# gpmp-dev/gpmp

Measured on AMD Instinct MI355X. Metric: fp64 predict+NLL throughput (points/s) and potrf TFLOP/s vs roofline, n=32k, higher is better.
Workload: dtype f64

## Files before the change

gpmp_amd/csrc/common.h:

```cpp
#pragma once
#include <hip/hip_runtime.h>
#include <cstdint>
#include <cstdio>
#include <cstring>
#include <atomic>
#include <vector>
#include "../../include/gpmp_hip.h"

namespace gpmp {

typedef double d4 __attribute__((ext_vector_type(4)));
typedef double d2 __attribute__((ext_vector_type(2)));

constexpr int NB = GPMP_NB;
constexpr int OUTER_BLOCKS = 4;

void set_error(const char* fmt, ...);
int hip_fail(hipError_t e, const char* what);

#define GPMP_HIP_TRY(expr)                                   \
  do {                                                       \
    hipError_t e__ = (expr);                                 \
    if (e__ != hipSuccess) return ::gpmp::hip_fail(e__, #expr); \
  } while (0)

#define GPMP_ARG(cond, k, msg)                                          \
  do {                                                                  \
    if (!(cond)) { ::gpmp::set_error("argument %d: %s", (k), (msg)); return -(k); } \
  } while (0)

inline hipStream_t as_stream(gpmp_stream_t s) { return reinterpret_cast<hipStream_t>(s); }

hipError_t stage_vector(std::vector<double>* v, double* dst, hipStream_t st);

int device_cu_count();

struct DeviceOnce {
  std::atomic<unsigned long long> mask{0};
  long long need() {
    int dev = 0;
    if (hipGetDevice(&dev) != hipSuccess || dev < 0 || dev > 62) return -1;
    const unsigned long long bit = 1ull << dev;
    return (mask.load(std::memory_order_acquire) & bit) ? 0 : (long long)bit;
  }
  void done(long long bit) { mask.fetch_or((unsigned long long)bit, std::memory_order_release); }
};

enum ProfKind { PK_GEMM_NT = 0, PK_GEMM_NN = 1, PK_GEMM_TN = 2, PK_GEMM_TT = 3, PK_POTF2 = 4, PK_GRAM = 5,
                PK_COLDOTS = 6, PK_GRAD = 7, PK_GEMM2_NT = 8, PK_GEMM2_NN = 9, PK_GEMM2_TN = 10, PK_GEMM2_TT = 11,
                PK_COUNT = 12 };
extern bool g_prof_on;
void prof_start(int kind, hipStream_t st);
void prof_stop(int kind, hipStream_t st, double work);
struct ProfScope {
  int kind; hipStream_t st; double work; bool on;
  ProfScope(int k, hipStream_t s, double w) : kind(k), st(s), work(w), on(g_prof_on) { if (on) prof_start(kind, st); }
  ~ProfScope() { if (on) prof_stop(kind, st, work); }
};

struct GemmOpts {
  int lower_only = 0;
  int kstart_row = 0;
  int kend_row = 0;
  int kstart_col = 0;
  int kend_col = 0;
  int batch = 1;
  long stride_a = 0, stride_b = 0, stride_c = 0;
  int batch2 = 1;
  long stride2_a = 0, stride2_b = 0, stride2_c = 0;
  int lean = 0;
  int stair_num = 0, stair_den = 0, stair_off = 0, stair_sub = 0;
  int kg_rnum = 0, kg_rden = 0, kg_roff = 0, kg_cnum = 0, kg_cden = 0, kg_coff = 0;
};
int launch_gemm(bool a_kc, bool b_kc, int M, int N, int K, double alpha, const double* A, long lda,
                const double* B, long ldb, double beta, double* C, long ldc, const GemmOpts& o,
                hipStream_t st);

int launch_trsm_leaf_forward(const double* L, long ldl, const double* dinv_leaf, int nb, double* B, long ldb, int ncols,
                             double* G, hipStream_t st);

int launch_potf2_inv(double* A, long lda, int jb, double* dinv, int* info_dev, int offset, hipStream_t st);
int launch_potf2_inv_batch(double* A, long lda, int jb, double* dinv, int* info_dev, int offset, int nprob, long stride_a,
                           long stride_dinv, hipStream_t st);
int launch_trtri_blocks(const double* L, long ldl, int n, double* dinv, hipStream_t st);

constexpr int TRSV_FEW_MAX = 16;
int trsv_few(const double* L, int n, long ldl, const double* dinv, double* B, int m, long ldb, int trans,
             hipStream_t st);

int launch_tril(double* A, int n, long lda, hipStream_t st, int nprob = 1, long prob_stride = 0);
int launch_symmetrize(double* A, int n, long lda, hipStream_t st);
int launch_diag_blocks(double* T, int n, long ldt, const double* dinv, hipStream_t st, int nprob = 1, long prob_stride_t = 0,
                       long prob_stride_dinv = 0);

struct ProblemBatch {
  int nprob = 1;
  long stride_a = 0;
  long stride_dinv = 0;
};
int potrf_blocked_batch(double* A, int n, long lda, double* dinv, int* info_dev, const ProblemBatch& pb, hipStream_t st);
int trtri_doubling_batch(const double* L, int n, long ldl, const double* dinv, double* T, long ldt, const ProblemBatch& pb,
                         long stride_t, hipStream_t st);
int launch_gram_lower_batch(const double* x, long stride_x, const int* ns_dev, int nmax, int d, int p, const double* theta_host,
                            int noise, double diag_add, double* K, long ldk, long stride_k, int nprob, hipStream_t st,
                            const double* pp_dev = nullptr);
int gram_param_block_elems();
void fill_gram_param_block(double* blk, int d, int p, const double* theta, int noise, double diag_add);
int launch_grad_trace_batch(const double* Kinv, long ldk, long stride_kinv, const double* x, long stride_x, const int* ns_dev, int nmax,
                            int d, int p, const double* theta_host, int noise, const double* F, const double* G, int r, long ldf,
                            long stride_f, double* g_dev, double* ws, int nprob, hipStream_t st, const double* pp_dev = nullptr);
int lauum_lower_batch(const double* T, int n, long ldt, long stride_t, double* Kinv, long ldk, long stride_k, int nprob,
                      hipStream_t st);

}
```

gpmp_amd/csrc/gemm_f64.hip:

```cpp
#include "common.h"
#include <cstdlib>

namespace gpmp {

int g_machine_busy = 0;

namespace {

constexpr int BM = 128, BN = 128, BK = 16;
constexpr int LDK = 18;
constexpr int LDN = 144;
constexpr int TILE = 2304;
constexpr int NXCD = 8;
typedef unsigned int v4u __attribute__((ext_vector_type(4)));

struct GemmParams {
  const double* A;
  const double* B;
  double* C;
  long lda, ldb, ldc;
  int M, N, K;
  double alpha, beta;
  int lower_only, kstart_row, kend_row, kend_col;
  int kstart_col;
// ... 646 lines not shown
      const int k0 = kt * BK;
      double* sa = smem + buf * 2 * V2_TILE;
      double* sb = sa + V2_TILE;
#pragma unroll
      for (int s = 0; s < 4; ++s)
        __builtin_amdgcn_raw_ptr_buffer_load_lds(rsA, (lds_ptr)(sa + (wave * 32 + s * 8) * 16), 16, voffA[s & 1],
                                                 ((wave * 32 + s * 8) * (int)p.ldg + k0) * 8, 0, 0);
#pragma unroll
      for (int s = 0; s < 4; ++s)
        __builtin_amdgcn_raw_ptr_buffer_load_lds(rsB, (lds_ptr)(sb + (wave * 4 + s) * 128), 16, voffB[s & 1],
                                                 ((k0 + wave * 4 + s) * (int)p.ldb) * 8, 0, 0);
    };
    auto read_frags = [&](int ks, int buf) {
      const double* sa = smem + buf * 2 * V2_TILE;
      const double* sb = sa + V2_TILE;
#pragma unroll
      for (int i = 0; i < MI; ++i) fa[ks][i] = sa[v2_frag_addr<true>(wm + i * 16 + lr, ks * 4 + lk)];
#pragma unroll
      for (int j = 0; j < NJ; ++j) fb[ks][j] = sb[v2_frag_addr<false>(wn + j * 16 + lr, ks * 4 + lk)];
    };
    auto mfma_step = [&](int ks) {
#pragma unroll
      for (int i = 0; i < MI; ++i)
#pragma unroll
        for (int j = 0; j < NJ; ++j)
          acc[i][j] = __builtin_amdgcn_mfma_f64_16x16x4f64(fa[ks][i], fb[ks][j], acc[i][j], 0, 0, 0);
    };
#pragma unroll
    for (int i = 0; i < MI; ++i)
#pragma unroll
      for (int j = 0; j < NJ; ++j) acc[i][j] = (d4){0.0, 0.0, 0.0, 0.0};

    issue(0, 0);
    __syncthreads();
    read_frags(0, 0);
    read_frags(1, 0);
    for (int kt = 0; kt < nk; ++kt) {
      const int cur = kt & 1;
      const bool more = kt + 1 < nk;
      if (more) issue(kt + 1, cur ^ 1);
      read_frags(2, cur);
      __builtin_amdgcn_sched_barrier(0);
      mfma_step(0);
      __builtin_amdgcn_sched_barrier(0);
      read_frags(3, cur);
      __builtin_amdgcn_sched_barrier(0);
      mfma_step(1);
      mfma_step(2);
      __builtin_amdgcn_sched_barrier(0);
      __syncthreads();
      if (more) {
        read_frags(0, cur ^ 1);
        read_frags(1, cur ^ 1);
      }
      __builtin_amdgcn_sched_barrier(0);
      mfma_step(3);
    }
    double* cb = strip + (long)jb * BM * p.ldb;
    if (ncv == BNW) {
#pragma unroll
      for (int i = 0; i < MI; ++i)
#pragma unroll
        for (int r = 0; r < 4; ++r) {
          double* rp = cb + (long)(i * 16 + 4 * r) * p.ldb;
#pragma unroll
          for (int j = 0; j < NJ; ++j) rp[lane_off + j * 16] = acc[i][j][r];
        }
    } else {
#pragma unroll
      for (int i = 0; i < MI; ++i)
#pragma unroll
        for (int r = 0; r < 4; ++r) {
          double* rp = cb + (long)(i * 16 + 4 * r) * p.ldb;
#pragma unroll
          for (int j = 0; j < NJ; ++j)
            if (wn + j * 16 + lr < ncv) rp[lane_off + j * 16] = acc[i][j][r];
        }
    }
    __threadfence_block();
    __syncthreads();
  }
}

struct LeafGParams {
  const double* L;
  long ldl;
  const double* dinv;
  double* G;
  long ldg;
};

__global__ void __launch_bounds__(256) build_leaf_g_kernel(LeafGParams p) {
  const int jb = blockIdx.x, ib = blockIdx.y;
  if (ib > jb) return;
  const int t = threadIdx.x;
  const double* __restrict__ D = p.dinv + (size_t)jb * BM * BM;
  double* __restrict__ out = p.G + (long)jb * BM * p.ldg + ib * BN;
  if (ib == jb) {
    for (int e = t; e < BM * BN / 2; e += 256) {
      const int r = e / (BN / 2), c = (e % (BN / 2)) * 2;
      *reinterpret_cast<d2*>(out + (long)r * p.ldg + c) = *reinterpret_cast<const d2*>(D + r * BM + c);
    }
    return;
  }
  const double* __restrict__ Lb = p.L + (long)jb * BM * p.ldl + ib * BN;
  const int lane = t & 63, wave = t >> 6;
  const int wm = (wave >> 1) * 64, wn = (wave & 1) * 64;
  const int lr = lane & 15, lk = lane >> 4;
  d4 acc[4][4];
#pragma unroll
  for (int i = 0; i < 4; ++i)
#pragma unroll
    for (int j = 0; j < 4; ++j) acc[i][j] = (d4){0.0, 0.0, 0.0, 0.0};
  for (int k0 = 0; k0 < BM; k0 += 4) {
    double a[4], b[4];
#pragma unroll
    for (int i = 0; i < 4; ++i) a[i] = D[(wm + i * 16 + lr) * BM + k0 + lk];
#pragma unroll
    for (int j = 0; j < 4; ++j) b[j] = Lb[(long)(k0 + lk) * p.ldl + wn + j * 16 + lr];
#pragma unroll
    for (int i = 0; i < 4; ++i)
#pragma unroll
      for (int j = 0; j < 4; ++j) acc[i][j] = __builtin_amdgcn_mfma_f64_16x16x4f64(a[i], b[j], acc[i][j], 0, 0, 0);
  }
#pragma unroll
  for (int i = 0; i < 4; ++i)
#pragma unroll
    for (int r = 0; r < 4; ++r)
#pragma unroll
      for (int j = 0; j < 4; ++j)
        out[(long)(wm + i * 16 + lk + 4 * r) * p.ldg + wn + j * 16 + lr] = -acc[i][j][r];
}

constexpr int SBM = 32, SBN = 128, SLD = 18;

template <int SBMT>
__global__ void __launch_bounds__(256) gemm_nt_small_kernel(GemmParams p) {
  __shared__ __attribute__((aligned(16))) double sA[2][SBMT * SLD];
  __shared__ __attribute__((aligned(16))) double sB[2][SBN * SLD];
  const int row0 = blockIdx.y * SBMT, col0 = blockIdx.x * SBN;
  if (p.lower_only && col0 > row0 + SBMT - 1) return;
  __builtin_amdgcn_s_setprio(3);
  const int t = threadIdx.x, lane = t & 63;
  const int wave = __builtin_amdgcn_readfirstlane(t >> 6);
  const int wn = wave * 32;
  const int lr = lane & 15, lk = lane >> 4;
  const int srow = t >> 2, skq = (t & 3) * 4;
  const bool has_a = t < 4 * SBMT;
  int ar = row0 + (has_a ? srow : 0), br0 = col0 + srow, br1 = col0 + srow + 64;
  ar = ar < p.M ? ar : p.M - 1;
  br0 = br0 < p.N ? br0 : p.N - 1;
  br1 = br1 < p.N ? br1 : p.N - 1;
  const double* __restrict__ ap = p.A + (long)ar * p.lda + skq;
  const double* __restrict__ bp0 = p.B + (long)br0 * p.ldb + skq;
  const double* __restrict__ bp1 = p.B + (long)br1 * p.ldb + skq;

  constexpr int MI = SBMT / 16;
  d4 acc[MI][2];
#pragma unroll
  for (int i = 0; i < MI; ++i)
#pragma unroll
    for (int j = 0; j < 2; ++j) acc[i][j] = (d4){0.0, 0.0, 0.0, 0.0};

  const int nk = p.K / BK;
  for (int kc = 0; kc < nk; kc += 8) {
    const int cnt = (nk - kc) < 8 ? (nk - kc) : 8;
    d2 ra[8][2], rb[8][4];
#pragma unroll
    for (int q = 0; q < 8; ++q) {
      if (q < cnt) {
        const int ko = (kc + q) * BK;
        if (has_a) {
          ra[q][0] = *reinterpret_cast<const d2*>(ap + ko);
          ra[q][1] = *reinterpret_cast<const d2*>(ap + ko + 2);
        }
        rb[q][0] = *reinterpret_cast<const d2*>(bp0 + ko);
        rb[q][1] = *reinterpret_cast<const d2*>(bp0 + ko + 2);
// ... 123 lines not shown
          double v = alpha * acc[i][j][r];
          if (beta != 0.0) v += beta * *cp;
          *cp = v;
        }
      }
    }
}

#pragma clang diagnostic pop

template <bool AKC, bool BKC, bool CACC>
int launch_t(const GemmParams& p, hipStream_t st) {
  static DeviceOnce attr_once;
  const size_t lds = sizeof(double) * 4 * TILE;
  const size_t lds2 = sizeof(double) * 4 * V2_TILE;
  if (const long long dev_bit = attr_once.need()) {
    if (dev_bit < 0) { set_error("hipGetDevice failed or device ordinal above 62"); return -1; }
    GPMP_HIP_TRY(hipFuncSetAttribute(reinterpret_cast<const void*>(gemm_f64_kernel<AKC, BKC, CACC>),
                                     hipFuncAttributeMaxDynamicSharedMemorySize, (int)lds));
    GPMP_HIP_TRY(hipFuncSetAttribute(reinterpret_cast<const void*>(gemm_f64_kernel_v2<AKC, BKC, CACC>),
                                     hipFuncAttributeMaxDynamicSharedMemorySize, (int)lds2));
    GPMP_HIP_TRY(hipFuncSetAttribute(reinterpret_cast<const void*>(gemm_f64_kernel_v2<AKC, BKC, CACC, 112>),
                                     hipFuncAttributeMaxDynamicSharedMemorySize, (int)lds2));
    GPMP_HIP_TRY(hipFuncSetAttribute(reinterpret_cast<const void*>(gemm_f64_kernel_v2<AKC, BKC, CACC, 96>),
                                     hipFuncAttributeMaxDynamicSharedMemorySize, (int)lds2));
    attr_once.done(dev_bit);
  }
  static int use_v2 = -1;
  if (use_v2 < 0) { const char* e = getenv("GPMP_GEMM_V2"); use_v2 = e ? atoi(e) : 1; }
  const bool v2ok = use_v2 && p.K >= 512 && p.aligned && (p.M % 2 == 0) && (p.N % 2 == 0) && (p.K % BK == 0) && p.K > 0 &&
                    ((reinterpret_cast<uintptr_t>(p.C) & 15) == 0) && (p.ldc % 2 == 0) &&
                    (p.lda % 2 == 0) && (p.ldb % 2 == 0) && (p.ldc >= p.N) &&
                    ((long)BM * p.lda * 8 + (long)p.K * 8 < 0x7FFFFFFFL) && ((long)BN * p.ldb * 8 + (long)p.K * 8 < 0x7FFFFFFFL);
  GemmParams pf = p;
  if (v2ok && p.batch == 1 && p.batch2 == 1 && !p.lower_only && !p.stair_den && !(p.kstart_row | p.kend_row | p.kstart_col | p.kend_col | p.kg_rden | p.kg_cden) && p.N >= 16 * BN) {
    const long slots = 2L * device_cu_count();
    auto cost = [&](int w) { const long t = (long)p.tiles_m * ((p.N + w - 1) / w); return ((t + slots - 1) / slots) * (long)w; };
    long best = cost(BN);
    for (int w : {112, 96}) {
      const long c = cost(w);
      if (c * 100 < best * 97) { best = c; pf.bn = w; }
    }
    if (pf.bn != BN) {
      pf.tiles_n = (p.N + pf.bn - 1) / pf.bn;
      pf.ntiles = pf.tiles_m * pf.tiles_n;
    }
  }
  constexpr int small_max = 128;
  const bool lean_nt = p.batch == 1 && p.batch2 == 1 && AKC && BKC && p.lean && p.aligned && (p.K % BK == 0) && p.K >= BK && p.K <= 512 &&
                       !(p.kstart_row | p.kend_row | p.kstart_col | p.kend_col) && ((long)SBN * p.ldb * 8 + (long)p.K * 8 < 0x7FFFFFFFL) &&
                       ((long)SBM * p.lda * 8 + (long)p.K * 8 < 0x7FFFFFFFL);
  const bool small_nt = !lean_nt && p.batch == 1 && p.batch2 == 1 && AKC && BKC && p.aligned && (p.K % BK == 0) && p.K >= BK && p.K <= 512 &&
                        p.ntiles <= (p.K >= 512 ? 384 : small_max) && !(p.kstart_row | p.kend_row | p.kstart_col | p.kend_col);
  {
    const double kavg = (p.kstart_row || p.kend_row || p.kstart_col || p.kend_col || p.kg_rden || p.kg_cden) ? 0.5 * p.K : (double)p.K;
    ProfScope ps((AKC ? (BKC ? PK_GEMM_NT : PK_GEMM_NN) : (BKC ? PK_GEMM_TT : PK_GEMM_TN)) + ((v2ok && !small_nt) ? 8 : 0), st,
                 (!p.lower_only && !p.stair_den && !(p.kstart_row | p.kend_row | p.kstart_col | p.kend_col | p.kg_rden | p.kg_cden))
                     ? 2.0 * (double)p.M * (double)p.N * (double)p.K * p.batch * p.batch2
                     : 2.0 * (double)p.ntiles * BM * BN * kavg * p.batch * p.batch2);
    if (lean_nt) hipLaunchKernelGGL(gemm_nt_lean_kernel, dim3((p.N + SBN - 1) / SBN, (p.M + SBM - 1) / SBM), dim3(256), 0, st, p);
    else if (small_nt) {
      constexpr long below16 = 160;
      const long wg32 = (long)((p.N + SBN - 1) / SBN) * ((p.M + SBM - 1) / SBM);
      if (wg32 < below16) hipLaunchKernelGGL(gemm_nt_small_kernel<16>, dim3((p.N + SBN - 1) / SBN, (p.M + 15) / 16), dim3(256), 0, st, p);
      else hipLaunchKernelGGL(gemm_nt_small_kernel<SBM>, dim3((p.N + SBN - 1) / SBN, (p.M + SBM - 1) / SBM), dim3(256), 0, st, p);
    }
    else if (v2ok && pf.bn == 112) hipLaunchKernelGGL((gemm_f64_kernel_v2<AKC, BKC, CACC, 112>), dim3(pf.ntiles, pf.batch, pf.batch2), dim3(256), lds2, st, pf);
    else if (v2ok && pf.bn == 96) hipLaunchKernelGGL((gemm_f64_kernel_v2<AKC, BKC, CACC, 96>), dim3(pf.ntiles, pf.batch, pf.batch2), dim3(256), lds2, st, pf);
    else if (v2ok) hipLaunchKernelGGL((gemm_f64_kernel_v2<AKC, BKC, CACC>), dim3(p.ntiles, p.batch, p.batch2), dim3(256), lds2, st, p);
    else hipLaunchKernelGGL((gemm_f64_kernel<AKC, BKC, CACC>), dim3(p.ntiles, p.batch, p.batch2), dim3(256), lds, st, p);
  }
  GPMP_HIP_TRY(hipGetLastError());
  return 0;
}

template <bool AKC, bool BKC>
int launch_c(const GemmParams& p, hipStream_t st) {
  if (p.beta != 0.0 && p.alpha != 0.0) return launch_t<AKC, BKC, true>(p, st);
  return launch_t<AKC, BKC, false>(p, st);
}

}

int launch_trsm_leaf_forward(const double* L, long ldl, const double* dinv_leaf, int nb, double* B, long ldb, int ncols,
                             double* G, hipStream_t st) {
  if (ncols <= 0) return 0;
  const long ldg = (long)nb * BN;
  {
    LeafGParams g{L, ldl, dinv_leaf, G, ldg};
    hipLaunchKernelGGL(build_leaf_g_kernel, dim3(nb, nb), dim3(256), 0, st, g);
    GPMP_HIP_TRY(hipGetLastError());
  }
  static DeviceOnce attr_once;
  const size_t lds2 = sizeof(double) * 4 * V2_TILE;
  if (const long long dev_bit = attr_once.need()) {
    if (dev_bit < 0) { set_error("hipGetDevice failed or device ordinal above 62"); return -1; }
    GPMP_HIP_TRY(hipFuncSetAttribute(reinterpret_cast<const void*>(trsm_leaf_kernel<128>),
                                     hipFuncAttributeMaxDynamicSharedMemorySize, (int)lds2));
    GPMP_HIP_TRY(hipFuncSetAttribute(reinterpret_cast<const void*>(trsm_leaf_kernel<64>),
                                     hipFuncAttributeMaxDynamicSharedMemorySize, (int)lds2));
    GPMP_HIP_TRY(hipFuncSetAttribute(reinterpret_cast<const void*>(trsm_leaf_kernel<32>),
                                     hipFuncAttributeMaxDynamicSharedMemorySize, (int)lds2));
    GPMP_HIP_TRY(hipFuncSetAttribute(reinterpret_cast<const void*>(trsm_leaf_kernel<16>),
                                     hipFuncAttributeMaxDynamicSharedMemorySize, (int)lds2));
    GPMP_HIP_TRY(hipFuncSetAttribute(reinterpret_cast<const void*>(trsm_leaf_kernel<112>),
                                     hipFuncAttributeMaxDynamicSharedMemorySize, (int)lds2));
    GPMP_HIP_TRY(hipFuncSetAttribute(reinterpret_cast<const void*>(trsm_leaf_kernel<96>),
                                     hipFuncAttributeMaxDynamicSharedMemorySize, (int)lds2));
    GPMP_HIP_TRY(hipFuncSetAttribute(reinterpret_cast<const void*>(trsm_leaf_kernel<80>),
                                     hipFuncAttributeMaxDynamicSharedMemorySize, (int)lds2));
    attr_once.done(dev_bit);
  }
  constexpr int narrow_below = 192, min_strips = 256;
  const int strips128 = (ncols + BN - 1) / BN;
  int bnw = 128;
  if (strips128 < narrow_below) {
    bnw = 64;
    while (bnw > 16 && (ncols + bnw - 1) / bnw < min_strips) bnw >>= 1;
  } else {
    const int ncu = device_cu_count();
    auto cost = [&](int w) {
      const int sw = (ncols + w - 1) / w;
      const int L = (sw + ncu - 1) / ncu;
      return (double)w * (2.22 * (L / 2) + 1.25 * (L % 2));
    };
    double best = cost(128);
    for (int w : {112, 96, 80}) {
      const double c = cost(w);
      if (c < 0.97 * best) { best = c; bnw = w; }
    }
  }
  LeafSolveParams p{G, ldg, B, ldb, nb, ncols};
  ProfScope ps(PK_GEMM_NN, st, (double)ncols * (double)(nb * BM) * (double)((nb + 1) * BM));
  const dim3 grid((ncols + bnw - 1) / bnw);
  if (bnw == 128) hipLaunchKernelGGL(trsm_leaf_kernel<128>, grid, dim3(256), lds2, st, p);
  else if (bnw == 112) hipLaunchKernelGGL(trsm_leaf_kernel<112>, grid, dim3(256), lds2, st, p);
  else if (bnw == 96) hipLaunchKernelGGL(trsm_leaf_kernel<96>, grid, dim3(256), lds2, st, p);
  else if (bnw == 80) hipLaunchKernelGGL(trsm_leaf_kernel<80>, grid, dim3(256), lds2, st, p);
  else if (bnw == 64) hipLaunchKernelGGL(trsm_leaf_kernel<64>, grid, dim3(256), lds2, st, p);
  else if (bnw == 32) hipLaunchKernelGGL(trsm_leaf_kernel<32>, grid, dim3(256), lds2, st, p);
  else hipLaunchKernelGGL(trsm_leaf_kernel<16>, grid, dim3(256), lds2, st, p);
  GPMP_HIP_TRY(hipGetLastError());
  return 0;
}

static int launch_gemm_one(bool a_kc, bool b_kc, int M, int N, int K, double alpha, const double* A, long lda,
                           const double* B, long ldb, double beta, double* C, long ldc, const GemmOpts& o,
                           hipStream_t st) {
  if (M <= 0 || N <= 0) return 0;
  GemmParams p;
  p.A = A; p.B = B; p.C = C;
  p.lda = lda; p.ldb = ldb; p.ldc = ldc;
  p.M = M; p.N = N; p.K = K;
  p.alpha = alpha; p.beta = beta;
  p.lower_only = o.lower_only; p.kstart_row = o.kstart_row; p.kend_row = o.kend_row; p.kend_col = o.kend_col;
  p.kstart_col = o.kstart_col;
  p.tiles_m = (M + BM - 1) / BM;
  p.tiles_n = (N + BN - 1) / BN;
  p.stair_num = o.stair_num; p.stair_den = o.stair_den; p.stair_off = o.stair_off; p.stair_sub = o.stair_sub;
  p.kg_rnum = o.kg_rnum; p.kg_rden = o.kg_rden; p.kg_roff = o.kg_roff; p.kg_cnum = o.kg_cnum; p.kg_cden = o.kg_cden; p.kg_coff = o.kg_coff;
  if ((o.kg_rden > 0 || o.kg_cden > 0) && (o.lower_only | o.kstart_row | o.kend_row | o.kstart_col | o.kend_col)) {
    set_error("group contraction starts combined with another tile / k restriction");
    return -1;
  }
  if (o.stair_den > 0) {
    if (o.lower_only | o.kstart_row | o.kend_row | o.kstart_col | o.kend_col) { set_error("staircase tile set combined with another tile / k restriction"); return -1; }
    p.ntiles = 0;
    for (int g = 0; 8 * g < p.tiles_m; ++g) {
      const int gsize = (p.tiles_m - 8 * g) < 8 ? (p.tiles_m - 8 * g) : 8;
      p.ntiles += gsize * stair_cols(o.stair_num, o.stair_den, o.stair_off, o.stair_sub, p.tiles_n, g);
    }
    if (p.ntiles == 0) return 0;
  } else if (o.lower_only) {
    const int tn = p.tiles_n < p.tiles_m ? p.tiles_n : p.tiles_m;
    p.ntiles = tn * (tn + 1) / 2 + (p.tiles_m - tn) * tn;
// ... 46 lines not shown
```

gpmp_amd/csrc/linalg.hip:

```cpp
#include "common.h"
#include <vector>
#include <cstdlib>
#include <mutex>
#include <map>
#include <memory>
#include <thread>
#include <atomic>

namespace gpmp {
namespace {

inline int imin(int a, int b) { return a < b ? a : b; }
inline int imax(int a, int b) { return a > b ? a : b; }

int potrf_blocked(double* A, int n, long lda, double* dinv, int* info_dev, int row0, hipStream_t st,
                  const ProblemBatch* pb = nullptr) {
  const int nblk = (n + NB - 1) / NB;
  GemmOpts lower;
  lower.lower_only = 1;
  GemmOpts plain;
  GemmOpts scale;
  if (pb != nullptr && pb->nprob > 1) {
    lower.batch2 = plain.batch2 = scale.batch2 = pb->nprob;
    lower.stride2_a = lower.stride2_b = lower.stride2_c = pb->stride_a;
// ... 301 lines not shown
  }
  for (int k = 0; k + 1 < np; ++k) {
    const int p0 = pb[k], p1 = pb[k + 1], p2 = pb[k + 2];
    const int w = p1 - p0;
    hipStream_t sside = g_la.side;
    if (e_u2) GPMP_HIP_TRY(hipStreamWaitEvent(s1, e_u2, 0));
    const int lean_panel = (n - p2 >= LA_LEAN_ABOVE) ? 1 : 0;
    hipEvent_t e_main_go = e_f;
    ColsReady ready[2];
    int nready = 0;
    if (p2 - p1 == 2 * OUTER_BLOCKS * NB && p2 <= n && n - p1 > LA_SPLIT_ABOVE) {
      const int cuts[4] = {p1, p1 + NB, p1 + OUTER_BLOCKS * NB, p2};
      hipEvent_t e_panel = g_la.next();
      GPMP_HIP_TRY(hipEventRecord(e_panel, s1));
      GPMP_HIP_TRY(hipStreamWaitEvent(sside, e_panel, 0));
      if (e_u2) GPMP_HIP_TRY(hipStreamWaitEvent(sside, e_u2, 0));
      for (int q = 0; q < 3; ++q) {
        const int ca = cuts[q], cb = cuts[q + 1];
        hipStream_t sq = q == 0 ? s1 : sside;
        rc = launch_gemm(true, true, n - ca, cb - ca, w, -1.0, A + (long)ca * lda + p0, lda, A + (long)ca * lda + p0, lda,
                         1.0, A + (long)ca * lda + ca, lda, lower, sq);
        if (rc) return rc;
        if (q > 0) {
          ready[nready].col = ca;
          ready[nready].ev = g_la.next();
          GPMP_HIP_TRY(hipEventRecord(ready[nready].ev, sside));
          ++nready;
        }
      }
    } else {
      rc = launch_gemm(true, true, n - p1, p2 - p1, w, -1.0, A + (long)p1 * lda + p0, lda, A + (long)p1 * lda + p0, lda,
                       1.0, A + (long)p1 * lda + p1, lda, lower, s1);
      if (rc) return rc;
    }
    if (n - p1 <= LA_MAIN_AFTER_LA_BELOW) {
      e_main_go = g_la.next();
      GPMP_HIP_TRY(hipEventRecord(e_main_go, s1));
    }
    rc = factor_panel(A, n, lda, dinv, info_dev, p1, p2, s1, lean_panel, ready, nready);
    if (rc) return rc;
    const bool need_ef = sa != nullptr || k + 2 >= np || (n - p2 > LA_MAIN_AFTER_LA_BELOW);
    hipEvent_t e_f_next = e_f;
    if (need_ef) {
      e_f_next = g_la.next();
      GPMP_HIP_TRY(hipEventRecord(e_f_next, s1));
    }
    if (sa != nullptr && p2 == upd_end) {
      const int r0 = n1_solved;
      GPMP_HIP_TRY(hipStreamWaitEvent(g_solve_stream, e_f_next, 0));
      rc = trsm_forward(A + (long)r0 * lda + r0, p2 - r0, lda, dinv + (size_t)(r0 / NB) * NB * NB, sa->B + (long)r0 * sa->ldb,
                        sa->m, sa->ldb, sa->gws, g_solve_stream);
      if (rc) return rc;
      n1_solved = p2;
      rc = early_update(n1_solved);
      if (rc) return rc;
    }
    GPMP_HIP_TRY(hipStreamWaitEvent(s0, e_main_go, 0));
    if (p2 < n) {
      rc = launch_gemm(true, true, n - p2, n - p2, w, -1.0, A + (long)p2 * lda + p0, lda, A + (long)p2 * lda + p0, lda,
                       1.0, A + (long)p2 * lda + p2, lda, lower, s0);
      if (rc) return rc;
    }
    e_u2 = g_la.next();
    GPMP_HIP_TRY(hipEventRecord(e_u2, s0));
    e_f = e_f_next;
  }
  GPMP_HIP_TRY(hipStreamWaitEvent(s0, e_f, 0));
  if (sa != nullptr) {
    hipEvent_t e_rows = g_la.next();
    GPMP_HIP_TRY(hipEventRecord(e_rows, g_solve_stream));
    GPMP_HIP_TRY(hipStreamWaitEvent(s0, e_rows, 0));
  }
  return 0;
}

constexpr int POTRF_ONE_STREAM_MAX = 4 * OUTER_BLOCKS * NB;

int potrf_lower(double* A, int n, long lda, double* dinv, int* info_dev, hipStream_t st) {
  GPMP_HIP_TRY(hipMemsetAsync(info_dev, 0, sizeof(int), st));
  if (n <= POTRF_ONE_STREAM_MAX) return potrf_blocked(A, n, lda, dinv, info_dev, 0, st);
  return potrf_lookahead(A, n, lda, dinv, info_dev, st);
}

int trsm_forward(const double* L, int n, long ldl, const double* dinv, double* B, int m, long ldb, double* gws, hipStream_t st) {
  if (n <= LEAF_TRSM) {
    const bool ok = gws != nullptr && n % NB == 0 && m >= 4 * NB && (m % 2 == 0) && (ldb % 2 == 0) &&
                    ((reinterpret_cast<uintptr_t>(B) & 15) == 0) && ((long)n * ldb * 8 < 0x7FFFFFFFL);
    if (ok) return launch_trsm_leaf_forward(L, ldl, dinv, n / NB, B, ldb, m, gws, st);
    return trsm_forward_blocked(L, n, ldl, dinv, B, m, ldb, st);
  }
  const int n1 = split_point(n);
  int rc = trsm_forward(L, n1, ldl, dinv, B, m, ldb, gws, st);
  if (rc) return rc;
  GemmOpts plain;
  rc = launch_gemm(true, false, n - n1, m, n1, -1.0, L + (long)n1 * ldl, ldl, B, ldb, 1.0, B + (long)n1 * ldb, ldb, plain, st);
  if (rc) return rc;
  return trsm_forward(L + (long)n1 * ldl + n1, n - n1, ldl, dinv + (size_t)(n1 / NB) * NB * NB, B + (long)n1 * ldb, m, ldb, gws, st);
}

int trsm_backward(const double* L, int n, long ldl, const double* dinv, double* B, int m, long ldb, hipStream_t st) {
  if (n <= LEAF_TRSM) return trsm_backward_blocked(L, n, ldl, dinv, B, m, ldb, st);
  const int n1 = split_point(n);
  int rc = trsm_backward(L + (long)n1 * ldl + n1, n - n1, ldl, dinv + (size_t)(n1 / NB) * NB * NB, B + (long)n1 * ldb, m,
                         ldb, st);
  if (rc) return rc;
  GemmOpts plain;
  rc = launch_gemm(false, false, n1, m, n - n1, -1.0, L + (long)n1 * ldl, ldl, B + (long)n1 * ldb, ldb, 1.0, B, ldb, plain, st);
  if (rc) return rc;
  return trsm_backward(L, n1, ldl, dinv, B, m, ldb, st);
}

int trtri_doubling(const double* L, int n, long ldl, const double* dinv, double* T, long ldt, hipStream_t st,
                   const ProblemBatch* pb = nullptr, long stride_t = 0) {
  const int nprob = pb != nullptr ? pb->nprob : 1;
  const long sl = pb != nullptr ? pb->stride_a : 0;
  int rc = launch_diag_blocks(T, n, ldt, dinv, st, nprob, stride_t, pb != nullptr ? pb->stride_dinv : 0);
  if (rc) return rc;
  for (long s = NB; s < n; s *= 2) {
    const int npairs = (int)(n / (2 * s));
    const long tail0 = (long)npairs * 2 * s;
    for (int part = 0; part < 2; ++part) {
      const long o = part == 0 ? 0 : tail0;
      const int len2 = part == 0 ? (int)s : (int)(n - (tail0 + s));
      const int batch = part == 0 ? npairs : 1;
      if (batch <= 0 || len2 <= 0) continue;
      const double* T11 = T + o * ldt + o;
      const double* L21 = L + (o + s) * ldl + o;
      double* Wt = T + o * ldt + (o + s);
      double* T21 = T + (o + s) * ldt + o;
      const double* T22 = T + (o + s) * ldt + (o + s);
      if (part == 0) {
        double* W = Wt;
        GemmOpts g1;
        g1.kstart_col = 1;
        g1.batch = batch; g1.stride_a = 2 * s * (ldl + 1); g1.stride_b = 2 * s * (ldt + 1); g1.stride_c = 2 * s * (ldt + 1);
        g1.batch2 = nprob; g1.stride2_a = sl; g1.stride2_b = stride_t; g1.stride2_c = stride_t;
        rc = launch_gemm(true, false, len2, (int)s, (int)s, 1.0, L21, ldl, T11, ldt, 0.0, W, ldt, g1, st);
        if (rc) return rc;
        GemmOpts g2;
        g2.kend_row = 1;
        g2.batch = batch; g2.stride_a = g2.stride_b = g2.stride_c = 2 * s * (ldt + 1);
        g2.batch2 = nprob; g2.stride2_a = g2.stride2_b = g2.stride2_c = stride_t;
        rc = launch_gemm(true, false, len2, (int)s, len2, -1.0, T22, ldt, W, ldt, 0.0, T21, ldt, g2, st);
        if (rc) return rc;
        continue;
      }
      GemmOpts g1;
      g1.kstart_row = 1;
      g1.batch = batch; g1.stride_a = 2 * s * (ldt + 1); g1.stride_b = 2 * s * (ldl + 1); g1.stride_c = 2 * s * (ldt + 1);
      g1.batch2 = nprob; g1.stride2_a = stride_t; g1.stride2_b = sl; g1.stride2_c = stride_t;
      rc = launch_gemm(false, true, (int)s, len2, (int)s, 1.0, T11, ldt, L21, ldl, 0.0, Wt, ldt, g1, st);
      if (rc) return rc;
      GemmOpts g2;
      g2.kend_row = 1;
      g2.batch = batch; g2.stride_a = g2.stride_b = g2.stride_c = 2 * s * (ldt + 1);
      g2.batch2 = nprob; g2.stride2_a = g2.stride2_b = g2.stride2_c = stride_t;
      rc = launch_gemm(true, true, len2, (int)s, len2, -1.0, T22, ldt, Wt, ldt, 0.0, T21, ldt, g2, st);
      if (rc) return rc;
    }
  }
  return launch_tril(T, n, ldt, st, nprob, stride_t);
}

}

int potrf_blocked_batch(double* A, int n, long lda, double* dinv, int* info_dev, const ProblemBatch& pb, hipStream_t st) {
  GPMP_HIP_TRY(hipMemsetAsync(info_dev, 0, sizeof(int) * (size_t)pb.nprob, st));
  return potrf_blocked(A, n, lda, dinv, info_dev, 0, st, &pb);
}
int trtri_doubling_batch(const double* L, int n, long ldl, const double* dinv, double* T, long ldt, const ProblemBatch& pb,
                         long stride_t, hipStream_t st) {
  return trtri_doubling(L, n, ldl, dinv, T, ldt, st, &pb, stride_t);
}
int lauum_lower_batch(const double* T, int n, long ldt, long stride_t, double* Kinv, long ldk, long stride_k, int nprob,
                      hipStream_t st) {
  GemmOpts o;
  o.lower_only = 1;
  o.kstart_row = 1;
  o.batch2 = nprob; o.stride2_a = o.stride2_b = stride_t; o.stride2_c = stride_k;
  return launch_gemm(false, false, n, n, n, 1.0, T, ldt, T, ldt, 0.0, Kinv, ldk, o, st);
}
}

using namespace gpmp;

namespace gpmp {
namespace {
int release_device_state(int dev) {
  std::shared_ptr<DeviceState> ds;
  {
    std::lock_guard<std::mutex> lk(g_dev_table_mu);
    auto it = g_dev_table.find(dev);
    if (it == g_dev_table.end()) return 0;
    ds = std::move(it->second);
    g_dev_table.erase(it);
  }
  std::lock_guard<std::mutex> lk(ds->mu);
  hipError_t first = hipSuccess;
  auto note = [&](hipError_t e) { if (e != hipSuccess && first == hipSuccess) first = e; };
  for (hipStream_t* st : {&ds->la.helper, &ds->la.side, &ds->solve_stream})
    if (*st != nullptr) {
      note(hipStreamSynchronize(*st));
      note(hipStreamDestroy(*st));
      *st = nullptr;
    }
  for (hipEvent_t e : ds->la.pool) note(hipEventDestroy(e));
  ds->la.pool.clear();
  ds->la.used = 0;
  return first == hipSuccess ? 0 : hip_fail(first, "gpmp_device_release");
}
}
}

extern "C" int gpmp_device_state_count(void) {
  std::lock_guard<std::mutex> lk(g_dev_table_mu);
  return (int)g_dev_table.size();
}

extern "C" int gpmp_device_release(void) {
  int dev = 0;
  GPMP_HIP_TRY(hipGetDevice(&dev));
  return release_device_state(dev);
}

extern "C" int gpmp_debug_device_table_selftest(int threads, int ordinals, int iters) {
  GPMP_ARG(threads > 0 && threads <= 64, 1, "threads outside [1, 64]");
  GPMP_ARG(ordinals > 0 && ordinals <= 64, 2, "ordinals outside [1, 64]");
  const int before = gpmp_device_state_count();
  std::vector<std::vector<DeviceState*>> seen(threads, std::vector<DeviceState*>(ordinals, nullptr));
  std::atomic<int> bad{0};
  std::vector<std::thread> pool;
  for (int t = 0; t < threads; ++t)
    pool.emplace_back([&, t] {
      for (int it = 0; it < iters; ++it)
        for (int o = 0; o < ordinals; ++o) {
          const std::shared_ptr<DeviceState> ds = device_state(1000 + (o + t) % ordinals);
          std::lock_guard<std::mutex> lk(ds->mu);
          ds->la.used = 0;
          DeviceState*& slot = seen[t][(o + t) % ordinals];
          if (slot == nullptr) slot = ds.get();
          else if (slot != ds.get()) bad.fetch_add(1);
        }
    });
  for (auto& th : pool) th.join();
  for (int t = 1; t < threads; ++t)
    for (int o = 0; o < ordinals; ++o)
      if (seen[t][o] != seen[0][o]) bad.fetch_add(1);
  if (gpmp_device_state_count() != before + ordinals) bad.fetch_add(1);
  for (int o = 0; o < ordinals; ++o)
    if (release_device_state(1000 + o)) bad.fetch_add(1);
  if (gpmp_device_state_count() != before) bad.fetch_add(1);
  return bad.load();
}

extern "C" size_t gpmp_dinv_elems(int n) {
  if (n <= 0) return 0;
  return (size_t)((n + NB - 1) / NB) * NB * NB + (n > 2 * OUTER_BLOCKS * NB ? (size_t)4 * OUTER_BLOCKS * OUTER_BLOCKS * NB * NB : 0);
}

extern "C" int gpmp_potrf_lower_async(double* A, int n, long lda, double* dinv, int* info_dev,
                                      gpmp_stream_t stream) {
  GPMP_ARG(A != nullptr, 1, "A is NULL");
  GPMP_ARG(n >= 0 && n <= GPMP_MAX_EXTENT, 2, "n outside [0, GPMP_MAX_EXTENT]");
  GPMP_ARG(lda >= n, 3, "lda < n");
  GPMP_ARG(dinv != nullptr, 4, "dinv is NULL");
  GPMP_ARG(info_dev != nullptr, 5, "info is NULL");
  if (n == 0) return 0;
  return potrf_lower(A, n, lda, dinv, info_dev, as_stream(stream));
}

extern "C" int gpmp_potrf_trsm_lower_async(double* A, int n, long lda, double* dinv, int* info_dev, double* B, int m, long ldb,
                                           gpmp_stream_t stream) {
  GPMP_ARG(A != nullptr, 1, "A is NULL");
  GPMP_ARG(n >= 0 && n <= GPMP_MAX_EXTENT, 2, "n outside [0, GPMP_MAX_EXTENT]");
  GPMP_ARG(lda >= n, 3, "lda < n");
  GPMP_ARG(dinv != nullptr, 4, "dinv is NULL");
  GPMP_ARG(info_dev != nullptr, 5, "info_dev is NULL");
  GPMP_ARG(B != nullptr, 6, "B is NULL");
  GPMP_ARG(m >= 0 && m <= GPMP_MAX_EXTENT && ldb >= m, 8, "m outside [0, GPMP_MAX_EXTENT] or ldb < m");
  if (n == 0) return 0;
  hipStream_t st = as_stream(stream);
  GPMP_HIP_TRY(hipMemsetAsync(info_dev, 0, sizeof(int), st));
  double* gws = (n > 2 * OUTER_BLOCKS * NB) ? dinv + (size_t)((n + NB - 1) / NB) * NB * NB : nullptr;
  constexpr int along_above = 2 * OUTER_BLOCKS * NB, along_below = 8192;
  if (m > TRSV_FEW_MAX && n > along_above && n <= along_below) {
    SolveAlong sa;
    sa.B = B; sa.m = m; sa.ldb = ldb; sa.gws = gws;
    return potrf_lookahead(A, n, lda, dinv, info_dev, st, &sa);
  }
  int rc = (n <= POTRF_ONE_STREAM_MAX) ? potrf_blocked(A, n, lda, dinv, info_dev, 0, st) : potrf_lookahead(A, n, lda, dinv, info_dev, st);
  if (rc || m == 0) return rc;
  if (m <= TRSV_FEW_MAX) return trsv_few(A, n, lda, dinv, B, m, ldb, 0, st);
  return trsm_forward(A, n, lda, dinv, B, m, ldb, gws, st);
}

extern "C" int gpmp_trtri_diag_blocks(const double* L, int n, long ldl, double* dinv, gpmp_stream_t stream) {
  GPMP_ARG(L != nullptr, 1, "L is NULL");
  GPMP_ARG(n <= GPMP_MAX_EXTENT, 2, "n above GPMP_MAX_EXTENT");
  GPMP_ARG(ldl >= n, 3, "ldl < n");
  GPMP_ARG(dinv != nullptr, 4, "dinv is NULL");
  return launch_trtri_blocks(L, ldl, n, dinv, as_stream(stream));
}

extern "C" int gpmp_trsm_lower(const double* L, int n, long ldl, const double* dinv, double* B, int m,
                               long ldb, int trans, double* scratch, gpmp_stream_t stream) {
  GPMP_ARG(L != nullptr, 1, "L is NULL");
  GPMP_ARG(n >= 0 && n <= GPMP_MAX_EXTENT, 2, "n outside [0, GPMP_MAX_EXTENT]");
  GPMP_ARG(ldl >= n, 3, "ldl < n");
  GPMP_ARG(B != nullptr, 5, "B is NULL");
  GPMP_ARG(m >= 0 && m <= GPMP_MAX_EXTENT && ldb >= m, 7, "m outside [0, GPMP_MAX_EXTENT] or ldb < m");
  GPMP_ARG(dinv != nullptr || scratch != nullptr, 9, "dinv and scratch both NULL");
  if (n == 0 || m == 0) return 0;
  hipStream_t st = as_stream(stream);
  if (dinv == nullptr) {
    int rc = launch_trtri_blocks(L, ldl, n, scratch, st);
    if (rc) return rc;
    dinv = scratch;
  }
  if (m <= TRSV_FEW_MAX) return trsv_few(L, n, ldl, dinv, B, m, ldb, trans, st);
  double* gws = (scratch != nullptr && n > 2 * OUTER_BLOCKS * NB) ? scratch + (size_t)((n + NB - 1) / NB) * NB * NB : nullptr;
  return trans ? trsm_backward(L, n, ldl, dinv, B, m, ldb, st) : trsm_forward(L, n, ldl, dinv, B, m, ldb, gws, st);
}

extern "C" int gpmp_trsm_right_lower(const double* L, int k, long ldl, const double* dinv, double* B, int M, long ldb,
                                     gpmp_stream_t stream) {
  GPMP_ARG(L != nullptr, 1, "L is NULL");
  GPMP_ARG(k >= 0 && k <= GPMP_MAX_EXTENT && ldl >= k, 3, "k outside [0, GPMP_MAX_EXTENT] or ldl < k");
  GPMP_ARG(dinv != nullptr, 4, "dinv is NULL");
  GPMP_ARG(B != nullptr, 5, "B is NULL");
  GPMP_ARG(M >= 0 && M <= GPMP_MAX_EXTENT && ldb >= k, 7, "M outside [0, GPMP_MAX_EXTENT] or ldb < k");
  return trsm_right(L, k, ldl, dinv, B, M, ldb, as_stream(stream));
}

extern "C" int gpmp_trtri_lower(const double* L, int n, long ldl, const double* dinv, double* T, long ldt,
                                gpmp_stream_t stream) {
  GPMP_ARG(L != nullptr, 1, "L is NULL");
  GPMP_ARG(n <= GPMP_MAX_EXTENT, 2, "n above GPMP_MAX_EXTENT");
  GPMP_ARG(ldl >= n, 3, "ldl < n");
  GPMP_ARG(dinv != nullptr, 4, "dinv is NULL");
  GPMP_ARG(T != nullptr && ldt >= n, 5, "T is NULL or ldt < n");
// ... 30 lines not shown
```

Measured before the change: 44530.

## Build all TRSM leaf inverse blocks in one batched launch up front

Leaf G matrices (inverses of diagonal leaf blocks) were built one leaf at a time inside the recursive forward TRSM, each as a small serial launch sitting between GEMM updates. Now one batched launch over all leaves builds them before the recursion, and each leaf solve just indexes its slot. This removes many small serialized launches from the critical path but enlarges the workspace, since the dinv allocation now scales with the number of leaves.

Result: no change. 44680 (median of 5 runs) (+0.3%).

```diff
diff --git a/gpmp_amd/csrc/common.h b/gpmp_amd/csrc/common.h
--- a/gpmp_amd/csrc/common.h
+++ b/gpmp_amd/csrc/common.h
@@ -76,8 +76,8 @@
                 const double* B, long ldb, double beta, double* C, long ldc, const GemmOpts& o,
                 hipStream_t st);
 
-int launch_trsm_leaf_forward(const double* L, long ldl, const double* dinv_leaf, int nb, double* B, long ldb, int ncols,
-                             double* G, hipStream_t st);
+int launch_build_leaf_g(const double* L, long ldl, const double* dinv, int n, int leaf_a, int leaf_b, double* G, hipStream_t st);
+int launch_trsm_leaf_solve(const double* G, int leaf, int nb, double* B, long ldb, int ncols, hipStream_t st);
 
 int launch_potf2_inv(double* A, long lda, int jb, double* dinv, int* info_dev, int offset, hipStream_t st);
 int launch_potf2_inv_batch(double* A, long lda, int jb, double* dinv, int* info_dev, int offset, int nprob, long stride_a,
diff --git a/gpmp_amd/csrc/gemm_f64.hip b/gpmp_amd/csrc/gemm_f64.hip
--- a/gpmp_amd/csrc/gemm_f64.hip
+++ b/gpmp_amd/csrc/gemm_f64.hip
@@ -752,17 +752,29 @@
   }
 }
 
+constexpr int LEAF_BLOCKS = 4;
+constexpr long LEAF_G_SLOT = (long)LEAF_BLOCKS * BM * LEAF_BLOCKS * BN;
 struct LeafGParams {
   const double* L;
   long ldl;
   const double* dinv;
   double* G;
-  long ldg;
+  int n;
+  int leaf0;
 };
 
-__global__ void __launch_bounds__(256) build_leaf_g_kernel(LeafGParams p) {
+__global__ void __launch_bounds__(256) build_leaf_g_kernel(LeafGParams q) {
   const int jb = blockIdx.x, ib = blockIdx.y;
-  if (ib > jb) return;
+  const int leaf = q.leaf0 + (int)blockIdx.z;
+  const int left = (q.n - leaf * LEAF_BLOCKS * BM) / BM;
+  const int nb = left < LEAF_BLOCKS ? left : LEAF_BLOCKS;
+  if (ib > jb || jb >= nb) return;
+  struct { const double* L; long ldl; const double* dinv; double* G; long ldg; } p;
+  p.L = q.L + (long)leaf * LEAF_BLOCKS * BM * (q.ldl + 1);
+  p.ldl = q.ldl;
+  p.dinv = q.dinv + (size_t)leaf * LEAF_BLOCKS * BM * BM;
+  p.G = q.G + (long)leaf * LEAF_G_SLOT;
+  p.ldg = (long)nb * BN;
   const int t = threadIdx.x;
   const double* __restrict__ D = p.dinv + (size_t)jb * BM * BM;
   double* __restrict__ out = p.G + (long)jb * BM * p.ldg + ib * BN;
@@ -1052,15 +1064,18 @@
 
 }
 
-int launch_trsm_leaf_forward(const double* L, long ldl, const double* dinv_leaf, int nb, double* B, long ldb, int ncols,
-                             double* G, hipStream_t st) {
+int launch_build_leaf_g(const double* L, long ldl, const double* dinv, int n, int leaf_a, int leaf_b, double* G, hipStream_t st) {
+  if (leaf_b <= leaf_a) return 0;
+  LeafGParams g{L, ldl, dinv, G, n, leaf_a};
+  hipLaunchKernelGGL(build_leaf_g_kernel, dim3(LEAF_BLOCKS, LEAF_BLOCKS, leaf_b - leaf_a), dim3(256), 0, st, g);
+  GPMP_HIP_TRY(hipGetLastError());
+  return 0;
+}
+
+int launch_trsm_leaf_solve(const double* G, int leaf, int nb, double* B, long ldb, int ncols, hipStream_t st) {
   if (ncols <= 0) return 0;
+  G += (long)leaf * LEAF_G_SLOT;
   const long ldg = (long)nb * BN;
-  {
-    LeafGParams g{L, ldl, dinv_leaf, G, ldg};
-    hipLaunchKernelGGL(build_leaf_g_kernel, dim3(nb, nb), dim3(256), 0, st, g);
-    GPMP_HIP_TRY(hipGetLastError());
-  }
   static DeviceOnce attr_once;
   const size_t lds2 = sizeof(double) * 4 * V2_TILE;
   if (const long long dev_bit = attr_once.need()) {
diff --git a/gpmp_amd/csrc/linalg.hip b/gpmp_amd/csrc/linalg.hip
--- a/gpmp_amd/csrc/linalg.hip
+++ b/gpmp_amd/csrc/linalg.hip
@@ -407,20 +407,44 @@
   return potrf_lookahead(A, n, lda, dinv, info_dev, st);
 }
 
-int trsm_forward(const double* L, int n, long ldl, const double* dinv, double* B, int m, long ldb, double* gws, hipStream_t st) {
+struct LeafG {
+  const double* G = nullptr;
+  int a = 0, b = 0;
+};
+inline bool leaf_fusable(int rows, const double* B, int m, long ldb) {
+  return rows % NB == 0 && m >= 4 * NB && (m % 2 == 0) && (ldb % 2 == 0) && ((reinterpret_cast<uintptr_t>(B) & 15) == 0) &&
+         ((long)rows * ldb * 8 < 0x7FFFFFFFL);
+}
+
+int trsm_forward_rec(const double* L, int n, long ldl, const double* dinv, double* B, int m, long ldb, const LeafG& lg, int leaf0,
+                     hipStream_t st) {
   if (n <= LEAF_TRSM) {
-    const bool ok = gws != nullptr && n % NB == 0 && m >= 4 * NB && (m % 2 == 0) && (ldb % 2 == 0) &&
-                    ((reinterpret_cast<uintptr_t>(B) & 15) == 0) && ((long)n * ldb * 8 < 0x7FFFFFFFL);
-    if (ok) return launch_trsm_leaf_forward(L, ldl, dinv, n / NB, B, ldb, m, gws, st);
+    if (leaf0 >= lg.a && leaf0 < lg.b) return launch_trsm_leaf_solve(lg.G, leaf0, n / NB, B, ldb, m, st);
     return trsm_forward_blocked(L, n, ldl, dinv, B, m, ldb, st);
   }
   const int n1 = split_point(n);
-  int rc = trsm_forward(L, n1, ldl, dinv, B, m, ldb, gws, st);
+  int rc = trsm_forward_rec(L, n1, ldl, dinv, B, m, ldb, lg, leaf0, st);
   if (rc) return rc;
   GemmOpts plain;
   rc = launch_gemm(true, false, n - n1, m, n1, -1.0, L + (long)n1 * ldl, ldl, B, ldb, 1.0, B + (long)n1 * ldb, ldb, plain, st);
   if (rc) return rc;
-  return trsm_forward(L + (long)n1 * ldl + n1, n - n1, ldl, dinv + (size_t)(n1 / NB) * NB * NB, B + (long)n1 * ldb, m, ldb, gws, st);
+  return trsm_forward_rec(L + (long)n1 * ldl + n1, n - n1, ldl, dinv + (size_t)(n1 / NB) * NB * NB, B + (long)n1 * ldb, m, ldb, lg,
+                          leaf0 + n1 / LEAF_TRSM, st);
+}
+
+int trsm_forward(const double* L, int n, long ldl, const double* dinv, double* B, int m, long ldb, double* gws, hipStream_t st) {
+  LeafG lg;
+  if (gws != nullptr) {
+    const int nfull = n / LEAF_TRSM, last = n - nfull * LEAF_TRSM;
+    const bool full_ok = nfull > 0 && leaf_fusable(LEAF_TRSM, B, m, ldb);
+    const bool last_ok = last > 0 && leaf_fusable(last, B + (long)nfull * LEAF_TRSM * ldb, m, ldb);
+    lg.G = gws;
+    lg.a = full_ok ? 0 : nfull;
+    lg.b = last_ok ? nfull + 1 : (full_ok ? nfull : lg.a);
+    const int rc = launch_build_leaf_g(L, ldl, dinv, (n / NB) * NB, lg.a, lg.b, gws, st);
+    if (rc) return rc;
+  }
+  return trsm_forward_rec(L, n, ldl, dinv, B, m, ldb, lg, 0, st);
 }
 
 int trsm_backward(const double* L, int n, long ldl, const double* dinv, double* B, int m, long ldb, hipStream_t st) {
@@ -580,7 +604,8 @@
 
 extern "C" size_t gpmp_dinv_elems(int n) {
   if (n <= 0) return 0;
-  return (size_t)((n + NB - 1) / NB) * NB * NB + (n > 2 * OUTER_BLOCKS * NB ? (size_t)4 * OUTER_BLOCKS * OUTER_BLOCKS * NB * NB : 0);
+  const size_t leaves = (size_t)((n + LEAF_TRSM - 1) / LEAF_TRSM);
+  return (size_t)((n + NB - 1) / NB) * NB * NB + (n > 2 * OUTER_BLOCKS * NB ? leaves * LEAF_TRSM * LEAF_TRSM : 0);
 }
 
 extern "C" int gpmp_potrf_lower_async(double* A, int n, long lda, double* dinv, int* info_dev,
```
